# fxxJuses/MICFormer

Measured on AMD Instinct MI355X. Metric: train volumes/sec (128^3 CT+MRI pair), higher is better.
Workload: dtype bf16; 1 GPU; MicFormer base Head(embed_dim=48, depths 2-2-6-2, heads 3-6-12-24, window 2^3, 8 classes) full train step (fwd + MDiceLoss + bwd + Adam/cosine) on 128^3 CT+MR pairs, DropPath on; local_batch=2, global_batch=2, parallelism=dp1, launch=hipGraph replay (one graph)

## Files before the change

### include/micformer_hip.h

```cpp
#ifndef MICFORMER_HIP_H
#define MICFORMER_HIP_H

#include <stddef.h>
#include <stdint.h>

#ifdef __cplusplus
extern "C" {
#endif

typedef void* micf_stream_t;

#define MICF_OK 0
#define MICF_EINVAL (-1)
#define MICF_EUNSUPPORTED (-2)
#define MICF_ELAUNCH (-3)

#define MICF_ABI_VERSION 1

#define MICF_DTYPE_F32 0
#define MICF_DTYPE_BF16 1
#define MICF_DTYPE_BF16_ATTN_FP8 2

int micf_abi_version(void);
const char* micf_strerror(int code);
// ... 286 lines not shown
  const float* pre_x;
  const float *pre_mean, *pre_rstd;
  const float* pre_g;
  float* pre_part;
} micf_block_bwd_group;
int micf_block_recomputes_h(int C, int heads);
int micf_block_tile_tokens(int B, int D, int H, int W, int C, int heads, int hidden, int backward);
int micf_block_fwd_persistent_probe(const micf_block_fwd_group* groups, int ngroups, int B, int D, int H, int W, int C, int heads,
                                    int hidden, float eps, float scale, int dtype, int repeats, int* sync_ws, micf_stream_t stream);
int micf_probe_mfma_chain(const void* a, const void* b, const void* c, const void* d, float* out, int form, micf_stream_t stream);
typedef struct micf_weight_prep_item {
  const float* src;
  void* dst;
  void* dst_t;
  int32_t rows, cols, bf16 , reserved;
} micf_weight_prep_item;
int micf_weight_prep_grouped(const micf_weight_prep_item* items, int n, micf_stream_t stream);
int micf_block_fwd(const micf_block_fwd_group* groups, int ngroups, int B, int D, int H, int W, int C, int heads,
                   int hidden, float eps, float scale, int dtype, micf_stream_t stream);
int micf_block_bwd(const micf_block_bwd_group* groups, int ngroups, int B, int D, int H, int W, int C, int heads,
                   int hidden, float scale, int dtype, micf_stream_t stream);

int micf_zero(void* p, int64_t bytes, micf_stream_t stream);
int micf_drop_path_draw(void* rng, const float* keep, float* out, int n, int B, micf_stream_t stream);


int micf_grad_wire_pack(const float* src, int64_t n, void* dst, int64_t padded, micf_stream_t stream);
int micf_grad_wire_sum(const void* recv, int ranks, int64_t shard, void* out, micf_stream_t stream);
int micf_grad_wire_unpack(const void* src, float* dst, int64_t n, micf_stream_t stream);

// ... 5 lines not shown
```

### micformer_amd/_lib.py

```python
import ctypes
import os

_PKT = "DEBUG_CLR_GRAPH_PACKET_CAPTURE"
_pkt_before = os.environ.get(_PKT)
if os.environ.get("MICF_SEGMENTED", "0") == "1":
    os.environ.setdefault(_PKT, "0")

import torch

GRAPH_SEGMENTS_OK = os.environ.get(_PKT) == "0" and (_pkt_before == "0" or not torch.cuda.is_initialized())

_HERE = os.path.dirname(os.path.abspath(__file__))
LIB_PATH = os.environ.get("MICF_LIB") or os.path.join(_HERE, "libmicformer_hip.so")

_P, _I, _L, _F, _D = ctypes.c_void_p, ctypes.c_int, ctypes.c_int64, ctypes.c_float, ctypes.c_double
_T = {"p": _P, "i": _I, "l": _L, "f": _F, "d": _D}

SIGNATURES = {
    "micf_layernorm_fwd": "ppippppplifp",
    "micf_layernorm_bwd": "pppippppppplippp",
    "micf_layernorm_bwd_partial_rows": "lii",
    "micf_layernorm_bwd_finish": "pip",
    "micf_linear_fwd": "ppipppplppliiiip",
    "micf_linear_bwd_data": "pplppppiiliiip",
# ... 114 lines not shown
    FIELDS = ("x", "kvsrc", "ln1_g", "ln1_b", "bq", "bkv", "bp", "ln2_g", "ln2_b", "b1", "b2", "wq", "wkv", "wp", "w1", "w2",
              "s1", "s2", "y", "xn", "q", "kv", "o", "x1", "xn2", "h", "g", "stats", "kvs16", "hid", "samp_src", "ln16_g", "ln16_b", "w1c", "flow", "xs32",
              "nln_g", "nln_b", "nln_y", "nln_mean", "nln_rstd", "zero16")
    _fields_ = [(n, _VP) for n in FIELDS]


class BlockBwdGroup(ctypes.Structure):
    FIELDS = ("dy", "x", "x1", "stats", "q", "kv", "h", "ln1_g", "ln2_g", "wqt", "wkvt", "wpt", "w1t", "w2t", "s1", "s2",
              "dx", "dxs", "dx1", "dh", "dq", "dkv", "ln1_part", "ln2_part", "dx1_copy", "dy16", "xn2", "w1", "b1",
              "pre_d", "pre_x", "pre_mean", "pre_rstd", "pre_g", "pre_part")
    _fields_ = [(n, _VP) for n in FIELDS]


class WeightPrepItem(ctypes.Structure):
    _fields_ = [("src", _VP), ("dst", _VP), ("dst_t", _VP), ("rows", ctypes.c_int32), ("cols", ctypes.c_int32),
                ("bf16", ctypes.c_int32), ("reserved", ctypes.c_int32)]


class LnPairItem(ctypes.Structure):
    FIELDS = ("x", "gamma", "beta", "y", "mean", "rstd")
    _fields_ = [(n, _VP) for n in FIELDS]


class LnBwdPairItem(ctypes.Structure):
    FIELDS = ("dy", "x", "mean", "rstd", "gamma", "dx", "dgamma", "dbeta", "add", "partials")
    _fields_ = [(n, _VP) for n in FIELDS]


class OffsetHeadGroup(ctypes.Structure):
    FIELDS = ("xn", "xa", "conv_w", "conv_b", "conv_ws", "ln_g", "ln_b", "w1", "hid", "flow", "xs")
    _fields_ = [(n, _VP) for n in FIELDS]
# ... 190 lines not shown
```

### micformer_amd/csrc/loss_optim.hip

```cpp
#include "common.h"
#include "loss_terms.h"

namespace micf {

template <bool LABEL>
__global__ void __launch_bounds__(256) dice_bce_partial_kernel(const float* __restrict__ z, const void* __restrict__ tv,
                                                               double* __restrict__ sums, int K, int64_t V, int chunks) {
  const int plane = blockIdx.y;
  const int ch = plane % K;
  const int64_t per = (V + chunks - 1) / chunks;
  const int64_t v0 = blockIdx.x * per, v1 = (v0 + per < V) ? v0 + per : V;
  const float* zp = z + (int64_t)plane * V;
  const float* tp = static_cast<const float*>(tv) + (int64_t)plane * V;
  const uint8_t* lp8 = static_cast<const uint8_t*>(tv) + (int64_t)(plane / K) * V;
  LossAcc la{0.f, 0.f, 0.f, 0.f};
  const bool vec = !LABEL && (V & 3) == 0 && (per & 3) == 0 && ((reinterpret_cast<uintptr_t>(z) | reinterpret_cast<uintptr_t>(tv)) & 15) == 0;
  if (vec) {
    int64_t i = v0 + 4 * threadIdx.x;
    for (; i + 1024 < v1; i += 2048) {
      const float4 z4 = *reinterpret_cast<const float4*>(zp + i), t4 = *reinterpret_cast<const float4*>(tp + i);
      const float4 y4 = *reinterpret_cast<const float4*>(zp + i + 1024), u4 = *reinterpret_cast<const float4*>(tp + i + 1024);
      la.term(z4.x, t4.x); la.term(z4.y, t4.y); la.term(z4.z, t4.z); la.term(z4.w, t4.w);
      la.term(y4.x, u4.x); la.term(y4.y, u4.y); la.term(y4.z, u4.z); la.term(y4.w, u4.w);
    }
// ... 104 lines not shown
  const int wave = threadIdx.x >> 6;
  if ((threadIdx.x & 63) == 0) { part[wave][0] = a; part[wave][1] = b; part[wave][2] = c; }
  __syncthreads();
  if (threadIdx.x < 3) {
    const int q = threadIdx.x;
    atomicAdd(sums + plane * 3 + q, (double)part[0][q] + (double)part[1][q] + (double)part[2][q] + (double)part[3][q]);
  }
}
__global__ void dice_metric_final_kernel(const double* __restrict__ sums, float* __restrict__ out, int planes) {
  const int i = blockIdx.x * blockDim.x + threadIdx.x;
  if (i >= planes) return;
  const double I = sums[i * 3], P = sums[i * 3 + 1], T = sums[i * 3 + 2];
  out[i] = T == 0.0 ? (P == 0.0 ? 1.f : 0.f) : (float)((2.0 * I) / (P + T));
}

struct AdamState { long long step; double lr; };

__global__ void adam_tick_kernel(AdamState* st, double base_lr, double eta_min, long long t_max) {
  if (threadIdx.x != 0 || blockIdx.x != 0) return;
  st->step += 1;
  st->lr = eta_min + (base_lr - eta_min) * (1.0 + cos(3.14159265358979323846 * (double)(st->step - 1) / (double)t_max)) / 2.0;
}

__device__ __forceinline__ unsigned bf16_pair(float a, float b) {
  typedef __bf16 bf16x2_hw __attribute__((ext_vector_type(2)));
  typedef float f32x2_hw __attribute__((ext_vector_type(2)));
  const f32x2_hw f = {a, b};
  return __builtin_bit_cast(unsigned, __builtin_convertvector(f, bf16x2_hw));
}

__global__ void __launch_bounds__(256) adam_step_kernel(float* __restrict__ p, const float* __restrict__ g,
                                                        float* __restrict__ m, float* __restrict__ v, int64_t n,
                                                        const AdamState* __restrict__ st, float beta1, float beta2, float eps,
                                                        float gscale, uint16_t* __restrict__ p16) {
  const double step = (double)st->step;
  const float bc1 = (float)(1.0 - pow((double)beta1, step));
  const float bc2_sqrt = (float)sqrt(1.0 - pow((double)beta2, step));
  const float step_size = (float)(st->lr / (double)bc1);
  const int64_t stride = (int64_t)gridDim.x * 1024;
  for (int64_t i0 = ((int64_t)blockIdx.x * 256 + threadIdx.x) * 4; i0 < n; i0 += 2 * stride) {
    const int64_t i1 = i0 + stride;
    const bool full0 = i0 + 3 < n, full1 = i1 + 3 < n;
    float4 P[2], M[2], V[2], G[2];
    if (full0) { P[0] = *reinterpret_cast<float4*>(p + i0); M[0] = *reinterpret_cast<float4*>(m + i0); V[0] = *reinterpret_cast<float4*>(v + i0); G[0] = *reinterpret_cast<const float4*>(g + i0); }
    if (full1) { P[1] = *reinterpret_cast<float4*>(p + i1); M[1] = *reinterpret_cast<float4*>(m + i1); V[1] = *reinterpret_cast<float4*>(v + i1); G[1] = *reinterpret_cast<const float4*>(g + i1); }
#pragma unroll
    for (int h = 0; h < 2; ++h) {
      const int64_t i = h ? i1 : i0;
      if (i >= n) continue;
    if (h ? full1 : full0) {
      float* pp = &P[h].x; float* mm = &M[h].x; float* vv = &V[h].x; float* gg = &G[h].x;
#pragma unroll
      for (int e = 0; e < 4; ++e) {
        gg[e] *= gscale;
        mm[e] = mm[e] + (gg[e] - mm[e]) * (1.0f - beta1);
        vv[e] = vv[e] * beta2 + (1.0f - beta2) * gg[e] * gg[e];
        const float denom = sqrtf(vv[e]) / bc2_sqrt + eps;
        pp[e] = pp[e] - step_size * (mm[e] / denom);
      }
      *reinterpret_cast<float4*>(p + i) = P[h]; *reinterpret_cast<float4*>(m + i) = M[h]; *reinterpret_cast<float4*>(v + i) = V[h];
      if (p16) *reinterpret_cast<uint2*>(p16 + i) = make_uint2(bf16_pair(P[h].x, P[h].y), bf16_pair(P[h].z, P[h].w));
    } else {
      for (int64_t j = i; j < n; ++j) {
        const float gj = g[j] * gscale;
        m[j] = m[j] + (gj - m[j]) * (1.0f - beta1);
        v[j] = v[j] * beta2 + (1.0f - beta2) * gj * gj;
        p[j] = p[j] - step_size * (m[j] / (sqrtf(v[j]) / bc2_sqrt + eps));
        if (p16) p16[j] = (uint16_t)(bf16_pair(p[j], 0.f) & 0xFFFFu);
      }
    }
    }
  }
}

}
using namespace micf;

static int dice_fwd(const float* logits, const void* target, bool label, double* sums, float* loss, int B, int K, int64_t V,
                    hipStream_t s) {
  if (!logits || !target || !sums || !loss || B <= 0 || K <= 0 || V <= 0) return MICF_EINVAL;
  if (hipMemsetAsync(sums, 0, sizeof(double) * 4 * K, s) != hipSuccess) return MICF_ELAUNCH;
  int chunks = (int)((V + 32767) / 32768);
// ... 79 lines not shown
```

### micformer_amd/csrc/misc.hip

```cpp
#include <hip/hip_fp16.h>

#include "common.h"
#include <string.h>

namespace micf {

__global__ void __launch_bounds__(256) pad3d_kernel(const float* __restrict__ src, float* __restrict__ dst, int B, int D, int H,
                                                    int W, int Dp, int Hp, int Wp, int C, int64_t total) {
  for (int64_t i = (int64_t)blockIdx.x * 256 + threadIdx.x; i < total; i += (int64_t)gridDim.x * 256) {
    int64_t t = i / C; const int c = (int)(i - t * C);
    const int w = (int)(t % Wp); t /= Wp; const int h = (int)(t % Hp); t /= Hp; const int d = (int)(t % Dp); const int b = (int)(t / Dp);
    dst[i] = (d < D && h < H && w < W) ? src[((((int64_t)b * D + d) * H + h) * W + w) * C + c] : 0.f;
  }
}
__global__ void __launch_bounds__(256) crop3d_kernel(const float* __restrict__ src, float* __restrict__ dst, int B, int D, int H,
                                                     int W, int Dp, int Hp, int Wp, int C, int accumulate, int64_t total) {
  for (int64_t i = (int64_t)blockIdx.x * 256 + threadIdx.x; i < total; i += (int64_t)gridDim.x * 256) {
    int64_t t = i / C; const int c = (int)(i - t * C);
    const int w = (int)(t % W); t /= W; const int h = (int)(t % H); t /= H; const int d = (int)(t % D); const int b = (int)(t / D);
    const float v = src[((((int64_t)b * Dp + d) * Hp + h) * Wp + w) * C + c];
    dst[i] = accumulate ? dst[i] + v : v;
  }
}

// ... 251 lines not shown
    t[ty + j][4 * tx] = v.x; t[ty + j][4 * tx + 1] = v.y; t[ty + j][4 * tx + 2] = v.z; t[ty + j][4 * tx + 3] = v.w;
  }
  if (!a.dst_t[k]) return;
  __syncthreads();
#pragma unroll
  for (int j = 0; j < 64; j += 16) {
    const int c = c0 + ty + j, r = r0 + 4 * tx;
    const int valid = c < cols ? (rows - r < 4 ? rows - r : 4) : 0;
    if (valid <= 0) continue;
    const float4 v = make_float4(t[4 * tx][ty + j], t[4 * tx + 1][ty + j], t[4 * tx + 2][ty + j], t[4 * tx + 3][ty + j]);
    prep_store4(a.dst_t[k], at(c, r, rows), bf, valid == 4 && vr, valid, v);
  }
}
}

extern "C" int micf_weight_prep_grouped(const micf_weight_prep_item* items, int n, micf_stream_t stream) {
  if (n < 0 || (n > 0 && !items)) return MICF_EINVAL;
  for (int first = 0; first < n; first += micf::kPrepMax) {
    const int cnt = (n - first < micf::kPrepMax) ? n - first : micf::kPrepMax;
    micf::PrepArgs a;
    a.n = cnt;
    int blocks = 0;
    for (int k = 0; k < cnt; ++k) {
      const micf_weight_prep_item& it = items[first + k];
      const int align = (it.bf16 == 1 || it.bf16 == 2) ? 7 : 15;
      if (it.bf16 < 0 || it.bf16 > 3 || (it.bf16 >= 2 && ((it.rows | it.cols) & 15))) return MICF_EINVAL;
      if (!it.src || (!it.dst && !it.dst_t) || it.rows <= 0 || it.cols <= 0 || (reinterpret_cast<uintptr_t>(it.src) & 15) ||
          (reinterpret_cast<uintptr_t>(it.dst) & align) || (reinterpret_cast<uintptr_t>(it.dst_t) & align))
        return MICF_EINVAL;
      a.src[k] = it.src; a.dst[k] = it.dst; a.dst_t[k] = it.dst_t; a.rows[k] = it.rows; a.cols[k] = it.cols; a.bf16[k] = it.bf16;
      blocks += ((it.rows + 63) / 64) * ((it.cols + 63) / 64);
      a.end[k] = blocks;
    }
    hipLaunchKernelGGL(micf::weight_prep_kernel, dim3(blocks), dim3(256), 0, (hipStream_t)stream, a);
    if (hipGetLastError() != hipSuccess) return MICF_ELAUNCH;
  }
  return MICF_OK;
}

namespace micf {
constexpr int kSwMax = 64;
struct SwCoords { int n; int b[kSwMax], z[kSwMax], y[kSwMax], x[kSwMax]; };
// ... 190 lines not shown
```

### micformer_amd/engine.py

```python
import torch
import torch.distributed as dist

from . import _lib, ops
from .dist import FlatGradSync, OverlappedGradReduce, flatten_views, last_writer_per_bucket, module_buckets
from .loss.dice import MDiceLoss


class TrainEngine:
    def __init__(self, model, base_lr=1e-4, t_max=150, eta_min=0.0, betas=(0.9, 0.999), eps=1e-8, criterion=None,
                 use_graph=False, process_group=None, grad_bucket_bytes=64 << 20, parallel_modalities=True,
                 defer_wgrad=True, split_step=None, always_collective=False, flush_points=True, early_adam=True,
                 dp_graph_flushes=6, grad_bf16=None, segmented=None, uniform_batches=False):
        self.model = model
        self.criterion = criterion if criterion is not None else MDiceLoss()
        self.base_lr, self.t_max, self.eta_min = base_lr, t_max, eta_min
        self.betas, self.eps = betas, eps
        self.sync = FlatGradSync(process_group, grad_bucket_bytes, always=always_collective)
        self.world = self.sync.world
        self._flatten()
        self.sync.broadcast_params(self.flat_p)
        self.parallel_modalities = bool(parallel_modalities)
        self.defer_wgrad = bool(defer_wgrad)
        self.flush_points = bool(flush_points)
        self.early_adam = bool(early_adam)
# ... 82 lines not shown
            early = lambda n: root is not None and (n.startswith(root + ".patch_embed.") or any(
                n.startswith(f"{root}.layers.{i}.") for i in range(len(stages) - 1)))
            ends = [o + s for n, o, s in zip(names, offs, sizes) if early(n)]
            if ends:
                cut = (max(ends) + 3) // 4 * 4
                if all(o >= cut for n, o in zip(names, offs) if not early(n)) and cut < total:
                    self._early_cut, self._early_layer = cut, stages[len(stages) - 1]
        pick = lambda suffixes: [(n, p) for n, p in zip(names, params) if n.endswith(suffixes)]
        self._shadow_w = [(n, p) for n, p in pick(("attn.q.weight", "attn.kv.weight", "attn.proj.weight", "mlp.fc1.weight",
                                                   "mlp.fc2.weight"))
                          if p.dim() == 2 and min(p.shape) <= 384 and not ((p.shape[0] | p.shape[1]) & 15)]
        self._conv_w = [(n, p) for n, p in pick(("conv_offset.0.weight",)) if p.dim() == 5 and p.shape[0] <= 16]
        self._offset_of = {id(p): o for p, o in zip(params, offs)}
        self._prep_plans, self._shadow_bufs, self._prep_split = {}, {}, {}
        self._prep_stream = torch.cuda.Stream(device=dev)

    def _weight_prep(self):
        mode = ops.compute_dtype()
        plans = self._prep_plans.get(mode)
        if plans is None:
            ws = [p for _, p in self._shadow_w]
            offs, total = flatten_views(ws, align=8)
            fwd, spec = None, ops.shadow_spec(False)
            if spec is not None:
                buf = self._shadow_bufs[spec[0]] = torch.empty(max(total, 8), dtype=spec[2], device=self.flat_p.device)
                ftrip = []
                for p, o in zip(ws, offs):
                    setattr(p, spec[0], buf[o:o + p.numel()].view(p.shape))
                    ftrip.append((p.data, getattr(p, spec[0]), None))
                fwd = ops.WeightPrepPlan(ftrip, blocked=True)
            attr, transposed, dtype = ops.shadow_spec(True)
            buf = self._shadow_bufs[attr] = torch.empty(max(total, 8), dtype=dtype, device=self.flat_p.device)
            trip = []
            for p, o in zip(ws, offs):
                setattr(p, attr, buf[o:o + p.numel()].view(p.shape[1], p.shape[0]))
                trip.append((p.data, None, getattr(p, attr)))
            if "conv" not in self._shadow_bufs:
                ctrip = []
                for _, p in self._conv_w:
                    p._micf_c3f, p._micf_c3b = ops.conv3_prepared_like(p)
                    ctrip.append((p.data, p._micf_c3f, p._micf_c3b))
                self._shadow_bufs["conv"] = ops.Conv3PrepPlan(ctrip)
            plans = self._prep_plans[mode] = (fwd, ops.WeightPrepPlan(trip, blocked=True), self._shadow_bufs["conv"])
            cut = self._early_cut if self._early_cut is not None else self.flat_p.numel()
            late = lambda p: self._offset_of[id(p)] >= cut
            if fwd is not None:
                fe = ops.WeightPrepPlan([t for t, p in zip(ftrip, ws) if not late(p)], blocked=True)
                fl = ops.WeightPrepPlan([t for t, p in zip(ftrip, ws) if late(p)], blocked=True)
            else:
                fe = fl = None
            ctr = [(p.data, p._micf_c3f, p._micf_c3b) for _, p in self._conv_w]
            ce = ops.Conv3PrepPlan([t for t, (_, p) in zip(ctr, self._conv_w) if not late(p)])
            cl = ops.Conv3PrepPlan([t for t, (_, p) in zip(ctr, self._conv_w) if late(p)])
            self._prep_split[mode] = (fe, fl, ce, cl)
        return plans

    def _scoped_flags(self):
        import contextlib
        from . import functional as _fn
        from .models import MICFormer_self as _ms

        @contextlib.contextmanager
        def scope():
            prev = (_ms.PARALLEL_MODALITIES, self.ctx.defer_wgrad, self.ctx.flush_points, self.ctx.defer_calls, ops.ENGINE_SHADOWS)
            prev_fork, prev_lazy = _ms.FORK_AUTOGRAD_STREAMS, self.ctx.lazy_ln_ok
            self.ctx.lazy_ln_ok = _fn.LAZY_LN_DEFAULT
            _ms.FORK_AUTOGRAD_STREAMS = not (self.segmented and self.use_graph)
            prev_budget = self.ctx.flush_budget
            _ms.PARALLEL_MODALITIES, self.ctx.defer_wgrad = self.parallel_modalities, self.defer_wgrad
# ... 8 lines not shown
                self.ctx.flush_budget = prev_budget
                _ms.FORK_AUTOGRAD_STREAMS = prev_fork
                self.ctx.lazy_ln_ok = prev_lazy
        return scope()

    def _fwd_bwd(self, x, target, flush=True, carry_in=None, carry_out=False):
        from . import functional as _fn
        with _fn.use_context(self.ctx):
            return self._fwd_bwd_in_ctx(x, target, flush, carry_in, carry_out)

    def _fwd_bwd_in_ctx(self, x, target, flush, carry_in, carry_out):
        from . import functional as _fn
        _fn.drop_deferred()
        with self._scoped_flags():
            fwd, bwd, conv = self._weight_prep()
            main, side = torch.cuda.current_stream(), self._prep_stream
            _fn.clear_entry_hooks()
            carried = [None]
            if carry_in is not None:
                fe, _, ce, _ = self._prep_split[ops.compute_dtype()]
                ce.launch()
                if fe is not None:
                    side.wait_stream(main)
                    with torch.cuda.stream(side):
                        fe.launch()
                    _fn.park_entry_hook(lambda: main.wait_stream(side), at=1)
                carried = [None]

                def launch_carried_groups_segmented():
                    def group_work(grp):
                        def w():
                            _fn.launch_carried(carry_in.get(grp["key"], []))
                            for lo, hi in grp["ranges"]:
                                self._adam_range(lo, hi, 1.0)
                            fl, cl = self._carry_prep(grp)
                            cl.launch()
                            if fl is not None:
                                fl.launch()
                        return [w]

                    def prep():
                        ops.zero_(self.flat_g)
                        bwd.launch()
                    evs = self.ctx.segmenter.run_side_groups([group_work(g) for g in self._carry_groups] + [[prep]], keep=carry_in)
                    for grp, ev in zip(self._carry_groups, evs):
                        _fn.park_entry_hook((lambda e: (lambda: self.ctx.segmenter.wait(e)))(ev), at=grp["entry"], front=True)
                    carried[0] = evs[-1]

                def launch_carried_groups():
                    if self.ctx.segmenter is not None:
                        return launch_carried_groups_segmented()
                    wside = _fn._wgrad_stream(self.flat_p.device)
                    wside.wait_stream(main)
                    with torch.cuda.stream(wside):
                        for grp in self._carry_groups:
                            _fn.launch_carried(carry_in.get(grp["key"], []))
                            for lo, hi in grp["ranges"]:
                                self._adam_range(lo, hi, 1.0)
                            fl, cl = self._carry_prep(grp)
                            cl.launch()
                            if fl is not None:
                                fl.launch()
                            ev = torch.cuda.Event()
                            ev.record(wside)
                            _fn.park_entry_hook((lambda e: (lambda: main.wait_event(e)))(ev), at=grp["entry"])
                            carried[0] = ev
                    self.ctx.wside_used.add(self.flat_p.device)
                _fn.park_entry_hook(launch_carried_groups, at=3)
            else:
                conv.launch()
                if fwd is not None:
                    side.wait_stream(main)
                    with torch.cuda.stream(side):
                        fwd.launch()
                    _fn.park_entry_hook(lambda: main.wait_stream(side), at=1)

            def backward_prep():
                if carry_in is not None and self.ctx.segmenter is not None:
                    return
                side.wait_stream(main)
                if carried[0] is not None:
                    side.wait_event(carried[0])
                with torch.cuda.stream(side):
                    ops.zero_(self.flat_g)
                    bwd.launch()
            _fn.park_entry_hook(backward_prep, at=3)
            self.ctx.backward_hooks.clear()
            self._adam_tail_done = False
            full_flush = self.ctx.flush_points and self.ctx.flush_budget >= (1 << 30) and _fn.FLUSH_MAX_TOKENS >= (1 << 30)
            if carry_out:
                assert flush and self.world == 1 and self._early_cut is not None and full_flush
                self.ctx.carry["on"], self.ctx.carry["open"], self.ctx.carry["stash"] = True, True, []

                def close_carry():
                    self.ctx.carry["open"] = False
                    if self.ctx.segmenter is None:
                        self._side_anchor()
                self.ctx.backward_hooks[id(self._early_layer)] = close_carry
            elif flush and self.world == 1 and self._early_cut is not None and self.early_adam and full_flush:
                self.ctx.backward_hooks[id(self._early_layer)] = self._early_adam_segment if self.ctx.segmenter is not None else self._early_adam
# ... 36 lines not shown
                if cur or set(groups) - {g["key"] for g in self._carry_groups}:
                    raise RuntimeError("carried parameter-gradient batches do not map onto the stage groups")
                self._carried = groups
                self.ctx.carry["on"], self.ctx.carry["stash"] = False, []
        return loss.detach()

    def _adam(self, grad_scale):
        lo, hi = 0, self.flat_p.numel()
        if self._adam_tail_done:
            hi, self._adam_tail_done = self._early_cut, False
        else:
            ops.adam_tick(self.adam_state, self.base_lr, self.eta_min, self.t_max)
        self._adam_range(lo, hi, grad_scale)

    def _adam_range(self, lo, hi, grad_scale):
        ops.adam_step(self.flat_p[lo:hi], self.flat_g[lo:hi], self.flat_m[lo:hi], self.flat_v[lo:hi], self.adam_state,
                      self.betas[0], self.betas[1], self.eps, grad_scale=grad_scale)

    def _early_adam(self):
        from . import functional as _fn
        def tail():
            ops.adam_tick(self.adam_state, self.base_lr, self.eta_min, self.t_max)
            self._adam_range(self._early_cut, self.flat_p.numel(), 1.0)
        _fn.launch_pending_flush()
        dev = self.flat_p.device
        main, side = torch.cuda.current_stream(dev), _fn._wgrad_stream(dev)
        side.wait_stream(main)
        with torch.cuda.stream(side):
            tail()
        self.ctx.wside_used.add(dev)
        self._adam_tail_done = True

# ... 65 lines not shown
            ex = self._eager_exchange[mode] = self._exchange_for(buckets, [-1] * len(buckets))
        ex.reduce_all()

    def step(self, x, target):
        if not self.use_graph:
            loss = self._step_impl(x, target)
        elif self._graph is not None and not self._matches_static(x, target):
            loss = self._step_impl(x, target)
        else:
            if self._graph is None:
                self._capture(x, target)
            if x is not self._static[0]:
                self._static[0].copy_(x, non_blocking=True)
            if target is not self._static[1]:
                self._static[1].copy_(target, non_blocking=True)
            self._graph.replay()
            if self.split_step:
                self._flush_and_reduce(then_update=True)
            loss = self._static[2]
        self.steps_done += 1
        ops.PARAM_EPOCH[0] += 1
        return loss

    def _build_carry_groups(self):
        sw = getattr(self.model, "swin", None)
        layers, ups = getattr(sw, "layers", None), getattr(sw, "up_layers", None)
        if sw is None or layers is None or ups is None or self._early_cut is None or len(ups) != len(layers):
            return None
        n = len(layers)
        if n < 4:
            return None
        names = [nm for nm, _ in self.model.named_parameters()]
        root = "swin"
        spec = [(layers[n - 1], n, [f"{root}.layers.{n - 1}.", f"{root}.norm."])]
        for j in range(n):
            pre = [f"{root}.up_layers.{j}."]
# ... 12 lines not shown
                if ranges and lo <= ranges[-1][1]:
                    ranges[-1][1] = max(ranges[-1][1], hi)
                else:
                    ranges.append([lo, hi])
            ranges = [(lo, min(hi, self.flat_p.numel())) for lo, hi in ranges]
            groups.append({"key": id(mod), "entry": entry, "ranges": ranges, "params": {id(self.params[i]) for i in idx}})
        tail = {i for i, o in enumerate(self.offsets) if o >= self._early_cut}
        if seen != tail or self._early_layer is not layers[n - 1]:
            return None
        return groups

    def _carry_prep(self, grp):
        mode = ops.compute_dtype()
        cache = grp.setdefault("prep", {})
        if mode not in cache:
            _, fl_all, _, cl_all = self._prep_split[mode]
            mine = grp["params"]
            fl = None
            if fl_all is not None:
                fl = ops.WeightPrepPlan([t for t in fl_all.triples if id(self._owner_of(t[0])) in mine], blocked=True)
            cl = ops.Conv3PrepPlan([t for t in cl_all.triples if id(self._owner_of(t[0])) in mine])
            cache[mode] = (fl, cl)
        return cache[mode]

    def _owner_of(self, data):
        off = (data.data_ptr() - self.flat_p.data_ptr()) // 4
        return self._param_at[off]

    def step_many(self, xs, targets):
        k = len(xs)
        if self._carry_groups is None:
            self._carry_groups = self._build_carry_groups() or False
        from . import functional as _fn
        full_flush = (self.defer_wgrad and self.flush_points and not self.split_step and _fn.FLUSH_MAX_TOKENS >= (1 << 30))
        if k < 2 or not self.use_graph or self.world != 1 or not self._carry_groups or not full_flush:
            return self._step_by_step(xs, targets)
        ent = self._many
        if ent is not None and not (ent["k"] == k and ent["mode"] == ops.arith_mode() and all(
                x.shape == sx.shape and x.dtype == sx.dtype and type(x) is type(sx) and t.shape == st.shape and t.dtype == st.dtype
                for x, t, sx, st in zip(xs, targets, ent["x"], ent["t"]))):
            return self._step_by_step(xs, targets)
        if ent is None:
            ent = self._many = self._capture_many(xs, targets)
        for sx, x in zip(ent["x"], xs):
            sx.copy_(x, non_blocking=True)
        for st, t in zip(ent["t"], targets):
            st.copy_(t, non_blocking=True)
        ent["graph"].replay()
        self.steps_done += k
        ops.PARAM_EPOCH[0] += 1
        return list(ent["loss"])

    def _step_by_step(self, xs, targets):
        return [self.step(x, t).clone() for x, t in zip(xs, targets)]

    def _many_body(self, sxs, sts):
        losses, carry = [], None
        for i, (x, t) in enumerate(zip(sxs, sts)):
            last = i == len(sxs) - 1
            losses.append(self._fwd_bwd(x, t, carry_in=carry, carry_out=not last))
            if last:
                self._update()
                carry = None
            else:
                ops.adam_tick(self.adam_state, self.base_lr, self.eta_min, self.t_max)
# ... 14 lines not shown
                self._step_impl(sxs[0], sts[0])
                self._many_body(sxs, sts)
        finally:
            from . import functional as _fn0
            self.ctx.carry["on"], self.ctx.carry["open"], self.ctx.carry["stash"] = False, False, []
            torch.cuda.current_stream().wait_stream(side)
            torch.cuda.synchronize()
            with torch.no_grad():
                for dst, src in zip((self.flat_p, self.flat_m, self.flat_v, self.adam_state), keep):
                    dst.copy_(src)
                for dst, src in zip(dp_rng, dp_keep):
                    dst.copy_(src)
            torch.set_rng_state(rng_cpu)
            torch.cuda.set_rng_state(rng_dev, sxs[0].device)
            del keep
        if self.segmented:
            from . import functional as _fn
            torch.cuda.empty_cache()
            g = _fn.StepSegmenter(_fn._wgrad_stream(sxs[0].device))
            cs = torch.cuda.Stream(device=sxs[0].device)
            cs.wait_stream(torch.cuda.current_stream())
            with torch.cuda.stream(cs):
                self.ctx.segmenter = g
                try:
                    g.begin()
                    with torch.autograd.set_multithreading_enabled(False):
                        losses = self._many_body(sxs, sts)
                    g.finish()
                finally:
                    self.ctx.segmenter = None
# ... 32 lines not shown
        side = torch.cuda.Stream()
        side.wait_stream(torch.cuda.current_stream())
        with torch.cuda.stream(side):
            for _ in range(2):
                self._step_impl(sx, st)
        torch.cuda.current_stream().wait_stream(side)
        torch.cuda.synchronize()
        with torch.no_grad():
            for dst, src in zip((self.flat_p, self.flat_m, self.flat_v, self.adam_state), keep):
                dst.copy_(src)
            for dst, src in zip(dp_rng, dp_keep):
                dst.copy_(src)
        torch.set_rng_state(rng_cpu)
        torch.cuda.set_rng_state(rng_dev, sx.device)
        del keep
        body = (lambda: self._fwd_bwd(sx, st, flush=False)) if self.split_step else (lambda: self._step_impl(sx, st))
        if self.segmented:
            from . import functional as _fn
            torch.cuda.empty_cache()
            g = _fn.StepSegmenter(_fn._wgrad_stream(sx.device))
            cs = torch.cuda.Stream(device=sx.device)
            cs.wait_stream(torch.cuda.current_stream())
            with torch.cuda.stream(cs):
                self.ctx.segmenter = g
                try:
                    g.begin()
                    sl = body()
                    g.finish()
                finally:
                    self.ctx.segmenter = None
# ... 93 lines not shown
```

### micformer_amd/ops.py

```python
import ctypes

import torch

from . import _lib
from ._lib import call, f32, ptr


DETAIL = False

_COMPUTE_DTYPE = "fp32"


def compute_dtype():
    return _COMPUTE_DTYPE


def _dt():
    return 1 if _COMPUTE_DTYPE == "bf16" else 0


def set_compute_dtype(name):
    global _COMPUTE_DTYPE, _ATTN_FP8
    if name not in ("fp32", "bf16", "bf16+fp8attn"):
        raise ValueError("compute dtype must be 'fp32', 'bf16' or 'bf16+fp8attn'")
# ... 856 lines not shown
        self.triples = list(triples)
        self.n = len(self.triples)
        self.arr = (_lib.WeightPrepItem * max(self.n, 1))()
        self.nbytes = 0
        for it, (src, dst, dst_t) in zip(self.arr, self.triples):
            outs = [t for t in (dst, dst_t) if t is not None]
            assert outs and len({t.dtype for t in outs}) == 1 and outs[0].dtype in (torch.float32, torch.bfloat16)
            it.src, it.dst, it.dst_t, it.rows, it.cols = f32(src), ptr(dst), ptr(dst_t), src.shape[0], src.shape[1]
            it.bf16 = (2 if blocked else 1) if outs[0].dtype == torch.bfloat16 else (3 if blocked else 0)
            self.nbytes += src.numel() * (4 + sum(t.element_size() for t in outs))

    def launch(self):
        if self.n:
            call("micf_weight_prep_grouped", ctypes.cast(self.arr, ctypes.c_void_p), self.n,
                 cost=(self.nbytes, 0) if _lib.PROFILE is not None else None)


class Conv3PrepPlan:

    def __init__(self, triples):
        self.triples = list(triples)
        self.n = len(self.triples)
        self.arr = (_lib.Conv3PrepItem * max(self.n, 1))()
        for it, (w, fwd, bwd) in zip(self.arr, self.triples):
            it.w, it.fwd, it.bwd, it.N, it.Cin = f32(w), f32(fwd), f32(bwd), w.shape[0], w.shape[1]

    def launch(self):
        if self.n:
            call("micf_conv3_weight_prep_grouped", ctypes.cast(self.arr, ctypes.c_void_p), self.n)

# ... 306 lines not shown
```

Baseline: 233.9 pairs/s.

## Fuse Adam update with bf16 blocked weight shadow preparation

Adds an adam_prep kernel that applies the Adam update per 64x64 weight tile and writes the blocked bf16 forward and transposed shadow copies in the same pass. This removes the separate weight-prep pass that re-read the fp32 parameters after the optimizer step. Shadow refresh moves out of the captured graph and becomes stamp-based: it runs only when parameters change outside the fused path. The cost is more complex plan bookkeeping and an added dependency on shadow staleness detection being correct.

```diff
diff --git a/include/micformer_hip.h b/include/micformer_hip.h
--- a/include/micformer_hip.h
+++ b/include/micformer_hip.h
@@ -324,6 +324,10 @@
   void* dst;
   void* dst_t;
   int32_t rows, cols, bf16 , reserved;
+  const float* g; float* m; float* v;
+  const void* adam;
+  float beta1, beta2, eps, grad_scale;
+  int64_t tail;
 } micf_weight_prep_item;
 int micf_weight_prep_grouped(const micf_weight_prep_item* items, int n, micf_stream_t stream);
 int micf_block_fwd(const micf_block_fwd_group* groups, int ngroups, int B, int D, int H, int W, int C, int heads,
diff --git a/micformer_amd/_lib.py b/micformer_amd/_lib.py
--- a/micformer_amd/_lib.py
+++ b/micformer_amd/_lib.py
@@ -152,7 +152,9 @@
 
 class WeightPrepItem(ctypes.Structure):
     _fields_ = [("src", _VP), ("dst", _VP), ("dst_t", _VP), ("rows", ctypes.c_int32), ("cols", ctypes.c_int32),
-                ("bf16", ctypes.c_int32), ("reserved", ctypes.c_int32)]
+                ("bf16", ctypes.c_int32), ("reserved", ctypes.c_int32), ("g", _VP), ("m", _VP), ("v", _VP), ("adam", _VP),
+                ("beta1", ctypes.c_float), ("beta2", ctypes.c_float), ("eps", ctypes.c_float), ("grad_scale", ctypes.c_float),
+                ("tail", ctypes.c_int64)]
 
 
 class LnPairItem(ctypes.Structure):
diff --git a/micformer_amd/csrc/adam_math.h b/micformer_amd/csrc/adam_math.h
--- /dev/null
+++ b/micformer_amd/csrc/adam_math.h
@@ -0,0 +1,35 @@
+#pragma once
+#include <hip/hip_runtime.h>
+#include <stdint.h>
+
+namespace micf {
+
+struct AdamState { long long step; double lr; };
+
+struct AdamCoef { float bc2_sqrt, step_size; };
+
+__device__ __forceinline__ AdamCoef adam_coef(const AdamState* __restrict__ st, float beta1, float beta2) {
+  const double step = (double)st->step;
+  const float bc1 = (float)(1.0 - pow((double)beta1, step));
+  const float bc2_sqrt = (float)sqrt(1.0 - pow((double)beta2, step));
+  return AdamCoef{bc2_sqrt, (float)(st->lr / (double)bc1)};
+}
+
+__device__ __forceinline__ void adam_elem(float& p, float& m, float& v, float g, float gscale, float beta1, float beta2, float eps,
+                                          const AdamCoef c) {
+  g *= gscale;
+  m = m + (g - m) * (1.0f - beta1);
+  v = v * beta2 + (1.0f - beta2) * g * g;
+  const float denom = sqrtf(v) / c.bc2_sqrt + eps;
+  p = p - c.step_size * (m / denom);
+}
+
+__device__ __forceinline__ void adam_elem4(float4& p, float4& m, float4& v, float4 g, float gscale, float beta1, float beta2, float eps,
+                                           const AdamCoef c) {
+  adam_elem(p.x, m.x, v.x, g.x, gscale, beta1, beta2, eps, c);
+  adam_elem(p.y, m.y, v.y, g.y, gscale, beta1, beta2, eps, c);
+  adam_elem(p.z, m.z, v.z, g.z, gscale, beta1, beta2, eps, c);
+  adam_elem(p.w, m.w, v.w, g.w, gscale, beta1, beta2, eps, c);
+}
+
+}
diff --git a/micformer_amd/csrc/loss_optim.hip b/micformer_amd/csrc/loss_optim.hip
--- a/micformer_amd/csrc/loss_optim.hip
+++ b/micformer_amd/csrc/loss_optim.hip
@@ -1,5 +1,6 @@
 #include "common.h"
 #include "loss_terms.h"
+#include "adam_math.h"
 
 namespace micf {
 
@@ -142,7 +143,6 @@
   out[i] = T == 0.0 ? (P == 0.0 ? 1.f : 0.f) : (float)((2.0 * I) / (P + T));
 }
 
-struct AdamState { long long step; double lr; };
 
 __global__ void adam_tick_kernel(AdamState* st, double base_lr, double eta_min, long long t_max) {
   if (threadIdx.x != 0 || blockIdx.x != 0) return;
@@ -161,10 +161,7 @@
                                                         float* __restrict__ m, float* __restrict__ v, int64_t n,
                                                         const AdamState* __restrict__ st, float beta1, float beta2, float eps,
                                                         float gscale, uint16_t* __restrict__ p16) {
-  const double step = (double)st->step;
-  const float bc1 = (float)(1.0 - pow((double)beta1, step));
-  const float bc2_sqrt = (float)sqrt(1.0 - pow((double)beta2, step));
-  const float step_size = (float)(st->lr / (double)bc1);
+  const AdamCoef cf = adam_coef(st, beta1, beta2);
   const int64_t stride = (int64_t)gridDim.x * 1024;
   for (int64_t i0 = ((int64_t)blockIdx.x * 256 + threadIdx.x) * 4; i0 < n; i0 += 2 * stride) {
     const int64_t i1 = i0 + stride;
@@ -177,23 +174,14 @@
       const int64_t i = h ? i1 : i0;
       if (i >= n) continue;
     if (h ? full1 : full0) {
-      float* pp = &P[h].x; float* mm = &M[h].x; float* vv = &V[h].x; float* gg = &G[h].x;
-#pragma unroll
-      for (int e = 0; e < 4; ++e) {
-        gg[e] *= gscale;
-        mm[e] = mm[e] + (gg[e] - mm[e]) * (1.0f - beta1);
-        vv[e] = vv[e] * beta2 + (1.0f - beta2) * gg[e] * gg[e];
-        const float denom = sqrtf(vv[e]) / bc2_sqrt + eps;
-        pp[e] = pp[e] - step_size * (mm[e] / denom);
-      }
+      adam_elem4(P[h], M[h], V[h], G[h], gscale, beta1, beta2, eps, cf);
       *reinterpret_cast<float4*>(p + i) = P[h]; *reinterpret_cast<float4*>(m + i) = M[h]; *reinterpret_cast<float4*>(v + i) = V[h];
       if (p16) *reinterpret_cast<uint2*>(p16 + i) = make_uint2(bf16_pair(P[h].x, P[h].y), bf16_pair(P[h].z, P[h].w));
     } else {
       for (int64_t j = i; j < n; ++j) {
-        const float gj = g[j] * gscale;
-        m[j] = m[j] + (gj - m[j]) * (1.0f - beta1);
-        v[j] = v[j] * beta2 + (1.0f - beta2) * gj * gj;
-        p[j] = p[j] - step_size * (m[j] / (sqrtf(v[j]) / bc2_sqrt + eps));
+        float pj = p[j], mj = m[j], vj = v[j];
+        adam_elem(pj, mj, vj, g[j], gscale, beta1, beta2, eps, cf);
+        p[j] = pj; m[j] = mj; v[j] = vj;
         if (p16) p16[j] = (uint16_t)(bf16_pair(p[j], 0.f) & 0xFFFFu);
       }
     }
diff --git a/micformer_amd/csrc/misc.hip b/micformer_amd/csrc/misc.hip
--- a/micformer_amd/csrc/misc.hip
+++ b/micformer_amd/csrc/misc.hip
@@ -1,6 +1,7 @@
 #include <hip/hip_fp16.h>
 
 #include "common.h"
+#include "adam_math.h"
 #include <string.h>
 
 namespace micf {
@@ -289,8 +290,181 @@
 }
 }
 
+namespace micf {
+constexpr int kAdamPrepMax = 144;
+constexpr int kAdamTailChunk = 2048;
+struct AdamPrepArgs {
+  float* p;
+  int64_t dg, dm, dv;
+  void* dst; void* dst_t;
+  const AdamState* st;
+  float beta1, beta2, eps, gscale;
+  int n;
+  int end[kAdamPrepMax];
+  int src[kAdamPrepMax];
+  int so[kAdamPrepMax], to[kAdamPrepMax];
+  int dims[kAdamPrepMax];
+  int tail[kAdamPrepMax];
+};
+__device__ __forceinline__ int64_t k16_at(int r, int c, int Cn) {
+  return ((int64_t)(r >> 4) * (Cn >> 4) + (c >> 4)) * 256 + (r & 15) * 16 + (c & 15);
+}
+template <bool BF16>
+__device__ __forceinline__ void k16_store4(void* base, int64_t idx, float4 v) {
+  if (BF16) *reinterpret_cast<uint2*>(static_cast<uint16_t*>(base) + idx) = make_uint2(pack_bf16(v.x, v.y), pack_bf16(v.z, v.w));
+  else *reinterpret_cast<float4*>(static_cast<float*>(base) + idx) = v;
+}
+template <bool BF16>
+__global__ void __launch_bounds__(256) adam_prep_kernel(const AdamPrepArgs a) {
+  __shared__ float t[64][65];
+  const int w = blockIdx.x;
+  int k = 0, hi = a.n - 1;
+  while (k < hi) { const int mid = (k + hi) >> 1; if (w >= a.end[mid]) k = mid + 1; else hi = mid; }
+  const int local = w - (k ? a.end[k - 1] : 0);
+  const int rows = a.dims[k] >> 16, cols = a.dims[k] & 0xFFFF;
+  const int tc = (cols + 63) >> 6, tiles = ((rows + 63) >> 6) * tc;
+  float* __restrict__ p = a.p + a.src[k];
+  const float* __restrict__ g = p + a.dg;
+  float* __restrict__ m = p + a.dm;
+  float* __restrict__ v = p + a.dv;
+  const AdamCoef cf = adam_coef(a.st, a.beta1, a.beta2);
+  if (local >= tiles) {
+    const int64_t end = (int64_t)rows * cols + a.tail[k];
+    const int64_t i0 = (int64_t)rows * cols + (int64_t)(local - tiles) * kAdamTailChunk + 4 * threadIdx.x, i1 = i0 + 1024;
+    const bool full0 = i0 + 3 < end, full1 = i1 + 3 < end;
+    float4 P[2], M[2], V[2], G[2];
+    if (full0) { P[0] = *reinterpret_cast<float4*>(p + i0); M[0] = *reinterpret_cast<float4*>(m + i0); V[0] = *reinterpret_cast<float4*>(v + i0); G[0] = *reinterpret_cast<const float4*>(g + i0); }
+    if (full1) { P[1] = *reinterpret_cast<float4*>(p + i1); M[1] = *reinterpret_cast<float4*>(m + i1); V[1] = *reinterpret_cast<float4*>(v + i1); G[1] = *reinterpret_cast<const float4*>(g + i1); }
+#pragma unroll
+    for (int h = 0; h < 2; ++h) {
+      const int64_t i = h ? i1 : i0;
+      if (i >= end) continue;
+      if (h ? full1 : full0) {
+        adam_elem4(P[h], M[h], V[h], G[h], a.gscale, a.beta1, a.beta2, a.eps, cf);
+        *reinterpret_cast<float4*>(p + i) = P[h]; *reinterpret_cast<float4*>(m + i) = M[h]; *reinterpret_cast<float4*>(v + i) = V[h];
+      } else {
+        for (int64_t j = i; j < end; ++j) {
+          float pj = p[j], mj = m[j], vj = v[j];
+          adam_elem(pj, mj, vj, g[j], a.gscale, a.beta1, a.beta2, a.eps, cf);
+          p[j] = pj; m[j] = mj; v[j] = vj;
+        }
+      }
+    }
+    return;
+  }
+  const int r0 = (local / tc) * 64, c0 = (local % tc) * 64;
+  const int tx = threadIdx.x & 15, ty = threadIdx.x >> 4;
+  const int c = c0 + 4 * tx;
+  float4 P[4], M[4], V[4], G[4];
+#pragma unroll
+  for (int j = 0; j < 4; ++j) {
+    const int r = r0 + ty + 16 * j;
+    if (r < rows && c < cols) {
+      const int64_t i = (int64_t)r * cols + c;
+      P[j] = *reinterpret_cast<float4*>(p + i); M[j] = *reinterpret_cast<float4*>(m + i);
+      V[j] = *reinterpret_cast<float4*>(v + i); G[j] = *reinterpret_cast<const float4*>(g + i);
+    }
+  }
+  const int so = a.so[k], to = a.to[k];
+#pragma unroll
+  for (int j = 0; j < 4; ++j) {
+    const int r = r0 + ty + 16 * j;
+    if (r < rows && c < cols) {
+      const int64_t i = (int64_t)r * cols + c;
+      adam_elem4(P[j], M[j], V[j], G[j], a.gscale, a.beta1, a.beta2, a.eps, cf);
+      *reinterpret_cast<float4*>(p + i) = P[j]; *reinterpret_cast<float4*>(m + i) = M[j]; *reinterpret_cast<float4*>(v + i) = V[j];
+      if (so >= 0) k16_store4<BF16>(static_cast<char*>(a.dst) + (int64_t)so * (BF16 ? 2 : 4), k16_at(r, c, cols), P[j]);
+    } else {
+      P[j] = make_float4(0.f, 0.f, 0.f, 0.f);
+    }
+    t[ty + 16 * j][4 * tx] = P[j].x; t[ty + 16 * j][4 * tx + 1] = P[j].y; t[ty + 16 * j][4 * tx + 2] = P[j].z; t[ty + 16 * j][4 * tx + 3] = P[j].w;
+  }
+  if (to < 0) return;
+  __syncthreads();
+  void* dt = static_cast<char*>(a.dst_t) + (int64_t)to * (BF16 ? 2 : 4);
+#pragma unroll
+  for (int j = 0; j < 4; ++j) {
+    const int cc = c0 + ty + 16 * j, r = r0 + 4 * tx;
+    if (cc >= cols || r >= rows) continue;
+    const float4 q = make_float4(t[4 * tx][ty + 16 * j], t[4 * tx + 1][ty + 16 * j], t[4 * tx + 2][ty + 16 * j], t[4 * tx + 3][ty + 16 * j]);
+    k16_store4<BF16>(dt, k16_at(cc, r, rows), q);
+  }
+}
+
+static bool float_offset(const void* a, const void* b, int64_t& out) {
+  const int64_t d = (int64_t)(reinterpret_cast<intptr_t>(a) - reinterpret_cast<intptr_t>(b));
+  out = d / 4;
+  return (d & 3) == 0;
+}
+
+static int adam_prep_grouped(const micf_weight_prep_item* items, int n, hipStream_t stream) {
+  const micf_weight_prep_item& f = items[0];
+  int64_t dg, dm, dv;
+  if (!f.src || !f.g || !f.m || !f.v || (f.bf16 != 2 && f.bf16 != 3) || !float_offset(f.g, f.src, dg) ||
+      !float_offset(f.m, f.src, dm) || !float_offset(f.v, f.src, dv))
+    return MICF_EINVAL;
+  const bool bf = f.bf16 == 2;
+  const int esz = bf ? 2 : 4;
+  for (int first = 0; first < n; first += kAdamPrepMax) {
+    const int cnt = (n - first < kAdamPrepMax) ? n - first : kAdamPrepMax;
+    AdamPrepArgs a;
+    a.dg = dg; a.dm = dm; a.dv = dv;
+    a.st = static_cast<const AdamState*>(f.adam);
+    a.beta1 = f.beta1; a.beta2 = f.beta2; a.eps = f.eps; a.gscale = f.grad_scale;
+    a.n = cnt;
+    const char* pb = nullptr; const char* db = nullptr; const char* tb = nullptr;
+    for (int k = 0; k < cnt; ++k) {
+      const micf_weight_prep_item& it = items[first + k];
+      const char* s = reinterpret_cast<const char*>(it.src);
+      const char* d = static_cast<const char*>(it.dst);
+      const char* dt = static_cast<const char*>(it.dst_t);
+      if (s && (!pb || s < pb)) pb = s;
+      if (d && (!db || d < db)) db = d;
+      if (dt && (!tb || dt < tb)) tb = dt;
+    }
+    a.p = reinterpret_cast<float*>(const_cast<char*>(pb)); a.dst = const_cast<char*>(db); a.dst_t = const_cast<char*>(tb);
+    int64_t blocks = 0;
+    for (int k = 0; k < cnt; ++k) {
+      const micf_weight_prep_item& it = items[first + k];
+      int64_t d0, d1, d2, off;
+      if (!it.src || !it.g || !it.m || !it.v || it.adam != f.adam || it.bf16 != f.bf16 || it.beta1 != f.beta1 ||
+          it.beta2 != f.beta2 || it.eps != f.eps || it.grad_scale != f.grad_scale || !float_offset(it.g, it.src, d0) ||
+          !float_offset(it.m, it.src, d1) || !float_offset(it.v, it.src, d2) || d0 != dg || d1 != dm || d2 != dv ||
+          !aligned16(it.src) || !aligned16(it.g) || !aligned16(it.m) || !aligned16(it.v))
+        return MICF_EINVAL;
+      if (it.rows < 0 || it.cols < 0 || it.rows > 0x7FFF || it.cols > 0x7FFF || (it.rows == 0) != (it.cols == 0) ||
+          ((it.rows | it.cols) & 15) || it.tail < 0 || it.tail > (1 << 30) || (it.rows == 0 && it.tail == 0))
+        return MICF_EINVAL;
+      if (!float_offset(it.src, pb, off) || off > (1 << 30)) return MICF_EINVAL;
+      a.src[k] = (int)off;
+      a.so[k] = a.to[k] = -1;
+      if (it.rows > 0 && it.dst) {
+        const int64_t d = static_cast<const char*>(it.dst) - db;
+        if ((d % esz) || !aligned16(it.dst) || d / esz > (1 << 30)) return MICF_EINVAL;
+        a.so[k] = (int)(d / esz);
+      }
+      if (it.rows > 0 && it.dst_t) {
+        const int64_t d = static_cast<const char*>(it.dst_t) - tb;
+        if ((d % esz) || !aligned16(it.dst_t) || d / esz > (1 << 30)) return MICF_EINVAL;
+        a.to[k] = (int)(d / esz);
+      }
+      a.dims[k] = (it.rows << 16) | it.cols;
+      a.tail[k] = (int)it.tail;
+      blocks += (int64_t)((it.rows + 63) / 64) * ((it.cols + 63) / 64) + (it.tail + kAdamTailChunk - 1) / kAdamTailChunk;
+      if (blocks > (1 << 30)) return MICF_EINVAL;
+      a.end[k] = (int)blocks;
+    }
+    if (bf) hipLaunchKernelGGL(adam_prep_kernel<true>, dim3((unsigned)blocks), dim3(256), 0, stream, a);
+    else hipLaunchKernelGGL(adam_prep_kernel<false>, dim3((unsigned)blocks), dim3(256), 0, stream, a);
+    if (hipGetLastError() != hipSuccess) return MICF_ELAUNCH;
+  }
+  return MICF_OK;
+}
+}
+
 extern "C" int micf_weight_prep_grouped(const micf_weight_prep_item* items, int n, micf_stream_t stream) {
   if (n < 0 || (n > 0 && !items)) return MICF_EINVAL;
+  if (n > 0 && items[0].adam) return micf::adam_prep_grouped(items, n, (hipStream_t)stream);
   for (int first = 0; first < n; first += micf::kPrepMax) {
     const int cnt = (n - first < micf::kPrepMax) ? n - first : micf::kPrepMax;
     micf::PrepArgs a;
@@ -300,7 +474,7 @@
       const micf_weight_prep_item& it = items[first + k];
       const int align = (it.bf16 == 1 || it.bf16 == 2) ? 7 : 15;
       if (it.bf16 < 0 || it.bf16 > 3 || (it.bf16 >= 2 && ((it.rows | it.cols) & 15))) return MICF_EINVAL;
-      if (!it.src || (!it.dst && !it.dst_t) || it.rows <= 0 || it.cols <= 0 || (reinterpret_cast<uintptr_t>(it.src) & 15) ||
+      if (!it.src || it.adam || (!it.dst && !it.dst_t) || it.rows <= 0 || it.cols <= 0 || (reinterpret_cast<uintptr_t>(it.src) & 15) ||
           (reinterpret_cast<uintptr_t>(it.dst) & align) || (reinterpret_cast<uintptr_t>(it.dst_t) & align))
         return MICF_EINVAL;
       a.src[k] = it.src; a.dst[k] = it.dst; a.dst_t[k] = it.dst_t; a.rows[k] = it.rows; a.cols[k] = it.cols; a.bf16[k] = it.bf16;
diff --git a/micformer_amd/engine.py b/micformer_amd/engine.py
--- a/micformer_amd/engine.py
+++ b/micformer_amd/engine.py
@@ -120,6 +120,26 @@
         self._offset_of = {id(p): o for p, o in zip(params, offs)}
         self._prep_plans, self._shadow_bufs, self._prep_split = {}, {}, {}
         self._prep_stream = torch.cuda.Stream(device=dev)
+        self._adam_plans, self._shadow_stamp = {}, None
+
+    def _stamp(self):
+        return (ops.compute_dtype(), ops.PARAM_EPOCH[0], self.flat_p._version, sum(p._version for _, p in self._shadow_w))
+
+    def _shadows_current(self):
+        return self._shadow_stamp == self._stamp()
+
+    def _refresh_shadows(self):
+        fwd, bwd, _ = self._weight_prep()
+        for plan in (fwd, bwd):
+            if plan is not None:
+                plan.launch()
+        self._shadow_stamp = self._stamp()
+
+    def _bump_epoch(self):
+        fresh = self._shadows_current()
+        ops.PARAM_EPOCH[0] += 1
+        if fresh:
+            self._shadow_stamp = self._stamp()
 
     def _weight_prep(self):
         mode = ops.compute_dtype()
@@ -150,15 +170,10 @@
             plans = self._prep_plans[mode] = (fwd, ops.WeightPrepPlan(trip, blocked=True), self._shadow_bufs["conv"])
             cut = self._early_cut if self._early_cut is not None else self.flat_p.numel()
             late = lambda p: self._offset_of[id(p)] >= cut
-            if fwd is not None:
-                fe = ops.WeightPrepPlan([t for t, p in zip(ftrip, ws) if not late(p)], blocked=True)
-                fl = ops.WeightPrepPlan([t for t, p in zip(ftrip, ws) if late(p)], blocked=True)
-            else:
-                fe = fl = None
             ctr = [(p.data, p._micf_c3f, p._micf_c3b) for _, p in self._conv_w]
             ce = ops.Conv3PrepPlan([t for t, (_, p) in zip(ctr, self._conv_w) if not late(p)])
             cl = ops.Conv3PrepPlan([t for t, (_, p) in zip(ctr, self._conv_w) if late(p)])
-            self._prep_split[mode] = (fe, fl, ce, cl)
+            self._prep_split[mode] = (ce, cl)
         return plans
 
     def _scoped_flags(self):
@@ -197,16 +212,20 @@
         _fn.drop_deferred()
         with self._scoped_flags():
             fwd, bwd, conv = self._weight_prep()
+            prep = not self._shadows_current()
+            if prep:
+                self._shadow_stamp = self._stamp()
+            prep_shadows = prep
             main, side = torch.cuda.current_stream(), self._prep_stream
             _fn.clear_entry_hooks()
             carried = [None]
             if carry_in is not None:
-                fe, _, ce, _ = self._prep_split[ops.compute_dtype()]
+                ce, _ = self._prep_split[ops.compute_dtype()]
                 ce.launch()
-                if fe is not None:
+                if prep and fwd is not None:
                     side.wait_stream(main)
                     with torch.cuda.stream(side):
-                        fe.launch()
+                        fwd.launch()
                     _fn.park_entry_hook(lambda: main.wait_stream(side), at=1)
                 carried = [None]
 
@@ -216,15 +235,13 @@
                             _fn.launch_carried(carry_in.get(grp["key"], []))
                             for lo, hi in grp["ranges"]:
                                 self._adam_range(lo, hi, 1.0)
-                            fl, cl = self._carry_prep(grp)
-                            cl.launch()
-                            if fl is not None:
-                                fl.launch()
+                            self._carry_prep(grp).launch()
                         return [w]
 
                     def prep():
                         ops.zero_(self.flat_g)
-                        bwd.launch()
+                        if prep_shadows:
+                            bwd.launch()
                     evs = self.ctx.segmenter.run_side_groups([group_work(g) for g in self._carry_groups] + [[prep]], keep=carry_in)
                     for grp, ev in zip(self._carry_groups, evs):
                         _fn.park_entry_hook((lambda e: (lambda: self.ctx.segmenter.wait(e)))(ev), at=grp["entry"], front=True)
@@ -240,10 +257,7 @@
                             _fn.launch_carried(carry_in.get(grp["key"], []))
                             for lo, hi in grp["ranges"]:
                                 self._adam_range(lo, hi, 1.0)
-                            fl, cl = self._carry_prep(grp)
-                            cl.launch()
-                            if fl is not None:
-                                fl.launch()
+                            self._carry_prep(grp).launch()
                             ev = torch.cuda.Event()
                             ev.record(wside)
                             _fn.park_entry_hook((lambda e: (lambda: main.wait_event(e)))(ev), at=grp["entry"])
@@ -252,7 +266,7 @@
                 _fn.park_entry_hook(launch_carried_groups, at=3)
             else:
                 conv.launch()
-                if fwd is not None:
+                if prep and fwd is not None:
                     side.wait_stream(main)
                     with torch.cuda.stream(side):
                         fwd.launch()
@@ -266,7 +280,8 @@
                     side.wait_event(carried[0])
                 with torch.cuda.stream(side):
                     ops.zero_(self.flat_g)
-                    bwd.launch()
+                    if prep:
+                        bwd.launch()
             _fn.park_entry_hook(backward_prep, at=3)
             self.ctx.backward_hooks.clear()
             self._adam_tail_done = False
@@ -333,8 +348,19 @@
         self._adam_range(lo, hi, grad_scale)
 
     def _adam_range(self, lo, hi, grad_scale):
-        ops.adam_step(self.flat_p[lo:hi], self.flat_g[lo:hi], self.flat_m[lo:hi], self.flat_v[lo:hi], self.adam_state,
-                      self.betas[0], self.betas[1], self.eps, grad_scale=grad_scale)
+        key = (lo, hi, ops.compute_dtype(), float(grad_scale), tuple(self.betas), self.eps)
+        plan = self._adam_plans.get(key)
+        if plan is None:
+            self._weight_prep()
+            fa, ta = ops.shadow_spec(False), ops.shadow_spec(True)
+            mats = []
+            for _, p in self._shadow_w:
+                o = self._offset_of[id(p)]
+                if lo <= o < hi:
+                    mats.append((o, p.shape[0], p.shape[1], getattr(p, fa[0]) if fa is not None else None, getattr(p, ta[0])))
+            plan = self._adam_plans[key] = ops.AdamShadowPlan(self.flat_p, self.flat_g, self.flat_m, self.flat_v, lo, hi, mats,
+                                                              self.adam_state, self.betas[0], self.betas[1], self.eps, grad_scale)
+        plan.launch()
 
     def _early_adam(self):
         from . import functional as _fn
@@ -430,12 +456,14 @@
                 self._static[0].copy_(x, non_blocking=True)
             if target is not self._static[1]:
                 self._static[1].copy_(target, non_blocking=True)
+            if not self._shadows_current():
+                self._refresh_shadows()
             self._graph.replay()
             if self.split_step:
                 self._flush_and_reduce(then_update=True)
             loss = self._static[2]
         self.steps_done += 1
-        ops.PARAM_EPOCH[0] += 1
+        self._bump_epoch()
         return loss
 
     def _build_carry_groups(self):
@@ -478,13 +506,9 @@
         mode = ops.compute_dtype()
         cache = grp.setdefault("prep", {})
         if mode not in cache:
-            _, fl_all, _, cl_all = self._prep_split[mode]
+            _, cl_all = self._prep_split[mode]
             mine = grp["params"]
-            fl = None
-            if fl_all is not None:
-                fl = ops.WeightPrepPlan([t for t in fl_all.triples if id(self._owner_of(t[0])) in mine], blocked=True)
-            cl = ops.Conv3PrepPlan([t for t in cl_all.triples if id(self._owner_of(t[0])) in mine])
-            cache[mode] = (fl, cl)
+            cache[mode] = ops.Conv3PrepPlan([t for t in cl_all.triples if id(self._owner_of(t[0])) in mine])
         return cache[mode]
 
     def _owner_of(self, data):
@@ -510,9 +534,11 @@
             sx.copy_(x, non_blocking=True)
         for st, t in zip(ent["t"], targets):
             st.copy_(t, non_blocking=True)
+        if not self._shadows_current():
+            self._refresh_shadows()
         ent["graph"].replay()
         self.steps_done += k
-        ops.PARAM_EPOCH[0] += 1
+        self._bump_epoch()
         return list(ent["loss"])
 
     def _step_by_step(self, xs, targets):
@@ -557,6 +583,7 @@
             torch.set_rng_state(rng_cpu)
             torch.cuda.set_rng_state(rng_dev, sxs[0].device)
             del keep
+            self._refresh_shadows()
         if self.segmented:
             from . import functional as _fn
             torch.cuda.empty_cache()
@@ -619,6 +646,7 @@
         torch.set_rng_state(rng_cpu)
         torch.cuda.set_rng_state(rng_dev, sx.device)
         del keep
+        self._refresh_shadows()
         body = (lambda: self._fwd_bwd(sx, st, flush=False)) if self.split_step else (lambda: self._step_impl(sx, st))
         if self.segmented:
             from . import functional as _fn
diff --git a/micformer_amd/ops.py b/micformer_amd/ops.py
--- a/micformer_amd/ops.py
+++ b/micformer_amd/ops.py
@@ -894,6 +894,44 @@
         if self.n:
             call("micf_weight_prep_grouped", ctypes.cast(self.arr, ctypes.c_void_p), self.n,
                  cost=(self.nbytes, 0) if _lib.PROFILE is not None else None)
+
+
+class AdamShadowPlan:
+
+    def __init__(self, p, g, m, v, lo, hi, mats, state, beta1, beta2, eps, grad_scale):
+        items, cur = [], lo
+        for o, r, c, dst, dst_t in sorted(mats, key=lambda t: t[0]):
+            if o < cur or o + r * c > hi:
+                raise _lib.MicfError(f"AdamShadowPlan: matrix at {o} ({r} x {c}) overlaps another or leaves [{lo}, {hi})")
+            if o > cur:
+                if items:
+                    items[-1][5] += o - cur
+                else:
+                    items.append([cur, 0, 0, None, None, o - cur])
+            items.append([o, r, c, dst, dst_t, 0])
+            cur = o + r * c
+        if hi > cur:
+            if items:
+                items[-1][5] += hi - cur
+            else:
+                items.append([cur, 0, 0, None, None, hi - cur])
+        outs = [t for _, _, _, d, dt in mats for t in (d, dt) if t is not None]
+        assert len({t.dtype for t in outs}) <= 1 and all(t.dtype in (torch.float32, torch.bfloat16) for t in outs)
+        mode = 2 if outs and outs[0].dtype == torch.bfloat16 else 3
+        self.n = len(items)
+        self.arr = (_lib.WeightPrepItem * max(self.n, 1))()
+        bp, bg, bm, bv, st = f32(p), f32(g), f32(m), f32(v), ptr(state)
+        for it, (o, r, c, dst, dst_t, tail) in zip(self.arr, items):
+            it.src, it.g, it.m, it.v = bp + 4 * o, bg + 4 * o, bm + 4 * o, bv + 4 * o
+            it.dst, it.dst_t, it.rows, it.cols, it.bf16, it.tail = ptr(dst), ptr(dst_t), r, c, mode, tail
+            it.adam, it.beta1, it.beta2, it.eps, it.grad_scale = st, float(beta1), float(beta2), float(eps), float(grad_scale)
+        self.nbytes = 28 * (hi - lo) + sum(t.numel() * t.element_size() for t in outs)
+        self.flops = 12 * (hi - lo)
+
+    def launch(self):
+        if self.n:
+            call("micf_weight_prep_grouped", ctypes.cast(self.arr, ctypes.c_void_p), self.n,
+                 cost=(self.nbytes, self.flops) if _lib.PROFILE is not None else None)
 
 
 class Conv3PrepPlan:
```

After: 234.1 pairs/s, median of 6. About the same (+0.1%).
